# google/qhbm-library

Measured on AMD Instinct MI355X. Metric: circuit-expectation evals/sec (samples×Pauli terms) at n qubits; VQT step time, higher is better.
Workload: dtype f32; 1 GPU; BASELINE configs[2] (20-qubit XXZ, depth 16, 4096-sample VQT step): 20-qubit XXZ(delta=0.5) open chain, HEA depth 16 (944 params), 4096 states in total = 4096 on rank 0 of 1, VQT step = values + adjoint VJP; n_qubits=20, layers=16, states_total=4096, states_per_gpu=4096, pauli_terms=57, observables=1, hamiltonian=xxz, mode=vqt, parallelism=batch-sharded x1, backend_world_size=1, forward_passes=7, adjoint_passes=9

## Files before the change

qhbm-library_amd/csrc/engine.cpp:

```cpp
#include <hip/hip_runtime.h>

#include <algorithm>
#include <cmath>
#include <cstdio>
#include <iterator>
#include <cstdlib>
#include <cstring>
#include <memory>
#include <optional>
#include <string>
#include <vector>

#include "../../include/qhbm_engine.h"
#include "kernels.h"
#include "plan_args.h"
#include "program.h"
#include "schedule.h"

using namespace qhbm;

namespace {

std::string g_create_error;

// ... 55 lines not shown
};

struct TimedEvent {
  hipEvent_t a, b;
  int kind;
};

}

struct qhbm_engine {
  int device = -1;
  std::string err;
  Model model;
  bool have_circuit = false;
  int opt_tile = 0, opt_adj_tile = 0, opt_profile = 0, opt_round = 0;
  int opt_full_fwd = 60, opt_full_adj = 60, opt_force_general = 0;
  int opt_meas_tile = 0;
  int opt_values_from_obs = 1;
  bool retained_mu = false;
  int opt_cph_wave_bits = 1;
  int opt_fwd_values_obs = -1;
  int opt_adj_stop_early = -1;
  int opt_adj_plan_search = 1;
  int opt_wide_last = -1;
  int opt_fwd_pair = 1;
  int opt_shift_prefix = 1;
  int opt_adj_relabel = 1;
  int opt_obs_xcd_states = -1;
  int opt_x_two_shear = 1;
  int opt_adj_exchange = 1;
  int retained_U = 0;
  bool retained_table = false;
  int state_grad_U = 0;
  int64_t opt_chunk = 0;
  int64_t opt_budget_mb = 0;
  size_t resolved_budget = 0;
  bool plans_valid = false;
  bool adj_valid = false;
  std::vector<std::pair<std::vector<char>, std::unique_ptr<DevicePlan>>> adj_cache;
  int64_t fwd_plans_built = 0, adj_plans_built = 0;
  bool model_uploaded = false;
  DevicePlan fwd, adj;
  DevBuf<DevTerm> terms, global_terms;
  DevBuf<ObsGroup> obs_groups;
  bool terms_by_op = false;
  DevBuf<ObsBTerm> obs_bterms;
// ... 255 lines not shown

double pass_flops_per_amplitude(const Plan& plan, const Pass& p, const uint32_t* dyn = nullptr);

double adjoint_plan_seconds(const Plan& plan, const Model& m) {
  std::vector<PassArgs> args;
  std::vector<uint32_t> prog, tables;
  fill_args(plan, m, &args, &prog, &tables);
  const double amps = double(size_t(1) << plan.n_eff);
  double t = 0.0;
  for (size_t i = 0; i < args.size(); ++i) {
    const Pass& p = plan.passes[i];
    const double live = 1.0 / double(1ull << __builtin_popcount(args[i].zero_mask));
    int low_missing = 0;
    for (uint32_t k = 0; k < args[i].n_nonlocal; ++k) low_missing += args[i].nonlocal_pos[k] < 4;
    const double lines = std::min(1.0, live * double(1u << low_missing));
    const double write_share = (p.flags & PASS_RELABEL) ? 1.0 / double(1u << __builtin_popcount(p.frozen_new_local)) : 1.0;
    const double bytes = lines * amps * 8.0 * 2.0 * (1.0 + ((p.flags & PASS_STORE) ? write_share : 0.0));
    const double flops = live * amps * pass_flops_per_amplitude(plan, p);
    t += std::max(flops / 67e12, bytes / 5.5e12) + 0.1 * bytes / 5.5e12;
  }
  return t;
}

int build_plans(qhbm_engine* h) {
  if (h->plans_valid && h->adj_valid) return 0;
  if (!h->have_circuit) return fail(h, "qhbm_set_circuit has not been called");
  if (h->model.n_ops > kMaxOps) return fail(h, "too many observables (max 1024)");
  std::string err;
  if (!h->plans_valid) {
    h->adj_cache.clear();
    if (!build_plan(h->model, h->opt_tile, h->opt_round, false, &h->fwd.plan, &err, h->opt_full_fwd, h->opt_meas_tile,
                    h->opt_cph_wave_bits != 0, false, h->opt_wide_last))
      return fail(h, "forward plan: " + err);
    h->fwd.uploaded = false;
    ++h->fwd_plans_built;
  }
  const bool relabel = h->opt_adj_relabel != 0 && h->opt_adj_exchange != 0;
  auto plan_adjoint_of = [&](const Model& model, int tile, Plan* out, double* seconds, std::string* e) {
    if (!build_plan(model, tile, 0, true, out, e, h->opt_full_adj, 0, h->opt_cph_wave_bits != 0, relabel)) return false;
    *seconds = adjoint_plan_seconds(*out, model);
    if (!h->opt_adj_plan_search) return true;
    const std::vector<std::vector<uint32_t>> orders = out->candidate_orders;
    for (const std::vector<uint32_t>& order : orders) {
      Plan alt;
      std::string e2;
      if (!build_plan(model, tile, 0, true, &alt, &e2, h->opt_full_adj, 0, h->opt_cph_wave_bits != 0, relabel, -1, &order))
        continue;
      const double f = adjoint_plan_seconds(alt, model);
      if (std::getenv("QHBM_PLAN_DEBUG"))
        std::fprintf(stderr, "[plan] tile %d candidate with %zu passes: %.4g ms per state (kept so far: %zu passes, %.4g ms)\n", tile,
                     alt.passes.size(), f * 1e3, out->passes.size(), *seconds * 1e3);
      if (f < 0.99 * *seconds) { *out = std::move(alt); *seconds = f; }
    }
    return true;
  };
  auto plan_adjoint = [&](int tile, Plan* out, double* seconds, std::string* e) {
// ... 431 lines not shown
  HIPCHK(h->import_parts.reserve(import_norm_parts_count(n, c)));
  hipEvent_t* ev = timer_begin(h, 0, stream);
  HIPCHK(launch_import_states(h->import_src, n, n_eff, c, s0, h->psi.p, h->import_parts.p, h->import_norm2.p, stream));
  timer_end(ev, stream);
  if (h->import_upstream) {
    const size_t w = size_t(h->model.n_ops);
    HIPCHK(launch_scale_by_norm2(h->import_upstream + size_t(s0) * w, h->import_up.p + size_t(s0) * w, c, uint32_t(w),
                                 h->import_norm2.p + s0, stream));
  }
  return 0;
}

int run_forward_chunk(qhbm_engine* h, const int8_t* d_bits, uint32_t s0, uint32_t cs, bool keep_state,
                      hipStream_t stream, bool skip_measure = false) {
  DevicePlan& d = h->fwd;
  if (h->import_src)
    if (int rc = import_chunk(h, s0, cs, stream)) return rc;
  for (size_t i = 0; i < d.plan.passes.size(); ++i) {
    const Pass& p = d.plan.passes[i];
    if (skip_measure && p.is_measure_only) continue;
    const PassArgs a = forward_pass_args(h, i, keep_state, skip_measure);
    hipEvent_t* ev = timer_begin(h, 0, stream);
    const bool pair = h->opt_fwd_pair && cs >= 2 && !(a.flags & (PASS_INIT_BASIS | PASS_GENERAL)) && a.zero_mask == 0 &&
                      (skip_measure || p.n_meas_groups == 0) && pass_fwd_pair_supported(p.K);
    if (pair)
      HIPCHK(launch_pass_fwd_pair(p.K, a, cs, h->psi.p, d_bits, h->model.n, s0, d.prog.p, d.tables.p, d.coef.p, stream));
    else
      HIPCHK(launch_pass_fwd(p.K, d.plan.R, a, cs, h->psi.p, d_bits, h->model.n, d.prog.p, d.tables.p, d.coef.p,
                             h->op_scale.p, h->vals64.p, s0, stream));
    timer_end(ev, stream);
  }
  if (!d.plan.global_terms.empty() && !skip_measure)
    HIPCHK(launch_measure_global(h->psi.p, uint32_t(d.plan.n_eff), cs, h->global_terms.p,
                                 uint32_t(d.plan.global_terms.size()), h->op_scale.p, h->vals64.p,
                                 uint32_t(h->model.n_ops), s0, stream));
  return 0;
}

int values_begin(qhbm_engine* h, int U, hipStream_t stream) {
  const size_t nv = size_t(U) * size_t(std::max(h->model.n_ops, 1));
  HIPCHK(h->vals64.reserve(nv));
  HIPCHK(launch_zero_fill(h->vals64.p, nv * sizeof(unsigned long long), stream));
  return 0;
}
int values_end(qhbm_engine* h, int U, float* d_out, hipStream_t stream) {
  if (!d_out || h->model.n_ops <= 0) return 0;
// ... 500 lines not shown
  invalidate_plans(h);
  h->block_choice = -1;
  h->terms.release();
  return 0;
}

int qhbm_set_option(qhbm_engine* h, const char* name, int64_t value) {
  if (!h || !name) return 1;
  const std::string k(name);
  if (k == "tile_qubits") { h->opt_tile = int(value); invalidate_plans(h); h->block_choice = -1; }
  else if (k == "round_qubits") { h->opt_round = int(value); invalidate_plans(h); }
  else if (k == "force_general_kernels") h->opt_force_general = int(value);
  else if (k == "full_diag_threshold") { h->opt_full_fwd = int(value); invalidate_plans(h); }
  else if (k == "adjoint_full_diag_threshold") { h->opt_full_adj = int(value); invalidate_plans(h); }
  else if (k == "adjoint_tile_qubits") { h->opt_adj_tile = int(value); invalidate_plans(h); }
  else if (k == "adjoint_exchange") { h->opt_adj_exchange = int(value); invalidate_plans(h); }
  else if (k == "x_two_shear") { h->opt_x_two_shear = value != 0; invalidate_plans(h); h->adj_cache.clear(); h->dense.adj_cache.clear(); }
  else if (k == "adjoint_relabel") { h->opt_adj_relabel = int(value); invalidate_plans(h); }
  else if (k == "forward_pairs") h->opt_fwd_pair = int(value);
  else if (k == "shift_prefix_sharing") { h->opt_shift_prefix = int(value); h->shift_ready = false; }
  else if (k == "forward_values_from_observable") h->opt_fwd_values_obs = int(value);
  else if (k == "adjoint_stop_early") { h->opt_adj_stop_early = int(value); invalidate_plans(h); }
  else if (k == "adjoint_plan_search") { h->opt_adj_plan_search = int(value); invalidate_plans(h); }
  else if (k == "wide_last_pass") { h->opt_wide_last = int(value); invalidate_plans(h); }
  else if (k == "observable_xcd_states") h->opt_obs_xcd_states = int(value);
  else if (k == "observable_kernel") { h->opt_obs_kernel = int(value); h->block_choice = -1; }
  else if (k == "observable_split_rows") h->opt_obs_split_rows = value != 0;
  else if (k == "observable_block_bits") {
    if (value != kObsBlockBits && value != kObsBlockBitsSmall) return fail(h, "observable_block_bits: 12 or 13");
    h->opt_obs_block_bits = int(value); h->block_choice = -1; h->terms.release(); h->model_uploaded = false;
  }
  else if (k == "multi_observable_values") h->opt_multi_values = int(value);
  else if (k == "gather_multi_values") h->opt_gather_multi = int(value);
  else if (k == "observable_far_windows") { h->opt_far_windows = int(value); h->terms.release(); h->model_uploaded = false; }
  else if (k == "measure_tile_qubits") { h->opt_meas_tile = int(value); invalidate_plans(h); }
  else if (k == "values_from_observable") h->opt_values_from_obs = int(value);
  else if (k == "cph_wave_bits") { h->opt_cph_wave_bits = int(value); invalidate_plans(h); }
  else if (k == "chunk_states") h->opt_chunk = value;
  else if (k == "evolve_step_argument") {
    if (value < 1 || value > 64) return fail(h, "evolve_step_argument: 1 .. 64");
    h->opt_evolve_step = int(value);
  }
  else if (k == "workspace_budget_mb") h->opt_budget_mb = std::max<int64_t>(0, value);
  else if (k == "profile_events") h->opt_profile = int(value);
  else return fail(h, "unknown option '" + k + "'");
  return 0;
// ... 219 lines not shown
  if (int rc = prepare_coefs(h, d, d_params, -1, 0.0, s)) return rc;
  if (int rc = values_begin(h, U, s)) return rc;
  const uint32_t cs = chunk_states(h, U);
  if (int rc = ensure_state_buffers(h, cs, false)) return rc;
  const size_t row = size_t(8) << h->model.n, pitch = size_t(8) << d.plan.n_eff;
  for (uint32_t s0 = 0; s0 < uint32_t(U); s0 += cs) {
    const uint32_t c = std::min<uint32_t>(cs, uint32_t(U) - s0);
    if (int rc = h->model.gates.empty() ? import_chunk(h, s0, c, s) : run_forward_chunk(h, h->import_bits.p, s0, c, true, s)) return rc;
    char* out = static_cast<char*>(d_out_states) + size_t(s0) * row;
    HIPCHK(hipMemcpy2DAsync(out, row, h->psi.p, pitch, row, c, hipMemcpyDeviceToDevice, s));
    HIPCHK(launch_scale_state_rows(reinterpret_cast<float2*>(out), c, uint32_t(h->model.n), h->import_norm2.p + s0, s));
  }
  HIPCHK(h->phase_cs.reserve(2));
  HIPCHK(launch_global_phase(d.jobs.p, int(d.plan.jobs.size()), h->shift_phases.p, h->n_shift_phases, d_params,
                             h->phase_cs.p, s));
  HIPCHK(launch_scale_states(static_cast<float2*>(d_out_states), size_t(U) << h->model.n, h->phase_cs.p, s));
  return 0;
}

int qhbm_describe_schedule_from_states(qhbm_engine* h, char* buf, size_t buf_len) {
  if (!h || !buf || !buf_len) return 1;
  DenseScope scope(h);
  if (int rc = build_plans(h)) return rc;
  std::string s = describe_plan(h->fwd.plan) + describe_plan(h->adj.plan);
  char line[96];
  std::snprintf(line, sizeof(line), "adjoint time model: %.2f us per state\n", 1e6 * adjoint_plan_seconds(h->adj.plan, h->model));
  s += line;
  std::snprintf(buf, buf_len, "%s", s.c_str());
  return 0;
}

}

namespace {

struct EvolvePlan {
  double R = 0.0;
  int steps = 0;
  int terms = 0;
  double x = 0.0;
  std::vector<double> re, im;
};

std::vector<double> bessel_sequence(double x, int mode) {
  const int N = 2 * int(std::ceil(x)) + 64;
  std::vector<double> f(size_t(N) + 2, 0.0);
  f[size_t(N)] = 1.0;
// ... 746 lines not shown
  for (int k = 0; k < T; ++k) {
    for (size_t i = 0; i < nv; ++i) up[i] = (int(i % size_t(T)) == k) ? 1.f : 0.f;
    HIPCHK(hipMemcpyAsync(h->upstream_tmp.p, up.data(), nv * sizeof(float), hipMemcpyHostToDevice, s));
    HIPCHK(hipStreamSynchronize(s));
    if (int rc = adjoint_sweep(h, d_bits, U, d_params, h->upstream_tmp.p, d_out_vals, s)) return rc;
    HIPCHK(launch_scatter_jac(h->state_grad.p, uint32_t(U), uint32_t(h->adj.plan.slot_gate.size()),
                              h->param_slot_begin.p, h->param_slots.p, h->slot_factor.p, d_jac, uint32_t(T),
                              uint32_t(k), uint32_t(P), s));
  }
  return 0;
}

int qhbm_num_passes(qhbm_engine* h, int* forward_passes, int* backward_passes) {
  if (!h) return 1;
  if (int rc = build_plans(h)) return rc;
  if (forward_passes) *forward_passes = int(h->fwd.plan.passes.size());
  if (backward_passes) *backward_passes = int(h->adj.plan.passes.size());
  return 0;
}

int qhbm_describe_schedule(qhbm_engine* h, char* buf, size_t buf_len) {
  if (!h || !buf || !buf_len) return 1;
  if (int rc = build_plans(h)) return rc;
  std::string s = describe_plan(h->fwd.plan) + describe_plan(h->adj.plan);
  {
    char line[96];
    std::snprintf(line, sizeof(line), "adjoint time model: %.2f us per state\n", 1e6 * adjoint_plan_seconds(h->adj.plan, h->model));
    s += line;
  }
  if (!h->model.terms.empty()) {
    s += std::string("observable kernel: lambda = ") + (block_kernel(h) ? "observable_blocks_kernel" : "apply_observable_kernel");
    s += std::string(" values = ") + (gather_multi_mode(h) ? "apply_observable_kernel (an accumulator per observable)"
                                      : multi_value_mode(h) || (value_mode(h) && block_kernel(h)) ? "observable_blocks_kernel"
                                      : value_mode(h)                                            ? "apply_observable_kernel"
                                                                                                  : "measured in the passes");
    s += "\n";
  }
  std::snprintf(buf, buf_len, "%s", s.c_str());
  return 0;
}

int qhbm_kernel_time_ms(qhbm_engine* h, int reset, double* fwd_ms, int64_t* fwd_launches, double* bwd_ms,
                        int64_t* bwd_launches, double* obs_ms, int64_t* obs_launches) {
  if (!h) return 1;
  double ms[3] = {0.0, 0.0, 0.0};
  int64_t cnt[3] = {0, 0, 0};
  if (h->device >= 0 && !h->events.empty()) {
// ... 261 lines not shown
  if (obs_flops) *obs_flops = o;
  if (bwd_flops) *bwd_flops = b;
  return 0;
}

extern "C" {

int qhbm_traffic_model(qhbm_engine* h, int U, int with_vjp, double* fwd_bytes, double* obs_bytes,
                       double* bwd_bytes) {
  if (!h) return 1;
  if (int rc = build_plans(h)) return rc;
  const double tile_all = double(state_bytes(h)) * double(U);
  double f = 0.0, o = 0.0, b = 0.0;
  bool measure_only_after = !h->fwd.plan.global_terms.empty();
  for (const Pass& p : h->fwd.plan.passes) measure_only_after |= p.is_measure_only;
  const bool from_obs = with_vjp ? (value_mode(h) || multi_value_mode(h)) : forward_values_from_observable(h);
  {
    std::vector<PassArgs> fargs;
    std::vector<uint32_t> fprog, ftables;
    fill_args(h->fwd.plan, h->model, &fargs, &fprog, &ftables);
    for (size_t i = 0; i < fargs.size(); ++i) {
      const Pass& p = h->fwd.plan.passes[i];
      if (from_obs && p.is_measure_only) continue;
      const double live = 1.0 / double(1ull << __builtin_popcount(fargs[i].zero_mask));
      if (!(p.flags & PASS_INIT_BASIS)) f += live * tile_all;
      if (!p.is_measure_only && (!p.completes_circuit || from_obs || with_vjp || measure_only_after)) f += live * tile_all;
    }
  }
  if (!with_vjp && from_obs) o = tile_all;
  if (with_vjp) {
    o = 2.0 * tile_all;
    if (multi_value_mode(h) && !gather_multi_mode(h)) o += tile_all;
    std::vector<PassArgs> args;
    std::vector<uint32_t> prog, tables;
    fill_args(h->adj.plan, h->model, &args, &prog, &tables);
    for (size_t i = 0; i < args.size(); ++i) {
      double live = 1.0 / double(1ull << __builtin_popcount(args[i].zero_mask));
      {
        int low_missing = 0;
        for (uint32_t k = 0; k < args[i].n_nonlocal; ++k) low_missing += args[i].nonlocal_pos[k] < 4;
        live = std::min(1.0, live * double(1u << low_missing));
      }
      const Pass& ap = h->adj.plan.passes[i];
      double write_share = 1.0;
      if (ap.flags & PASS_RELABEL) write_share = 1.0 / double(1u << __builtin_popcount(ap.frozen_new_local));
      b += live * tile_all * 2.0 * (1.0 + ((ap.flags & PASS_STORE) ? write_share : 0.0));
    }
// ... 9 lines not shown
```

qhbm-library_amd/csrc/kernels.hip:

```cpp
#include <hip/hip_runtime.h>
#include <stdint.h>
#include <cstdio>
#include <cstring>

#include <utility>

#include "../../include/qhbm_engine.h"
#include "device_common.h"
#include "kernels.h"
#include "program.h"
#include "x_shear.h"

namespace qhbm {

namespace {


__device__ __forceinline__ uint32_t swz(uint32_t l) { return l ^ ((l >> 5) & 31u); }

constexpr int wg_per_cu(int lds_bytes) { return (160 * 1024) / lds_bytes < 1 ? 1 : (160 * 1024) / lds_bytes; }
constexpr int clampi(int v, int lo, int hi) { return v < lo ? lo : (v > hi ? hi : v); }
constexpr int fwd_lds(int K) { return (8 << K) + 8 * kMaxOps; }
constexpr int adj_lds(int K) { return (16 << K) + 4 * kMaxSlotsPerPass * ((1 << (K - 4)) / 64 < 1 ? 1 : (1 << (K - 4)) / 64); }
constexpr int adjx_lds(int K) { return (8 << K) + 4 * kMaxSlotsPerPass * ((1 << (K - 4)) / 64 < 1 ? 1 : (1 << (K - 4)) / 64); }
// ... 887 lines not shown
  wht_lane_stage<3>(w, lane);
  wht_lane_stage<4>(w, lane);
  wht_lane_stage<5>(w, lane);
  uint32_t begin = 0;
#pragma unroll
  for (int c = 0; c < NR; ++c) {
    const uint32_t end = uni(class_end[c]);
    if (end != begin) {
      scr[lane] = w[c];
      for (uint32_t k = begin + uint32_t(lane); k < end; k += 64u) {
        const uint32_t* tw = terms + size_t(k) * kMeasTermWords;
        const uint4 t = make_uint4(tw[0], tw[1], tw[2], tw[3]);
        const uint32_t par = uint32_t(__popc(tile_base & t.y) + __popc(wave & (t.x >> 6))) & 1u;
        const float v = __uint_as_float(t.z ^ (par << 31)) * scr[t.x & 63u];
        atomicAdd(&red[t.w], to_fixed(v, op_scale[t.w]));
      }
    }
    begin = end;
  }
}

}

template <int K, int R, bool GEN>
__global__ __launch_bounds__(1 << (K - R), fwd_min_waves(K, R)) void pass_fwd_kernel(
    PassArgs a, float2* __restrict__ psi, const int8_t* __restrict__ bits, int n_user,
    const uint32_t* __restrict__ prog_base, const uint32_t* __restrict__ tables,
    const float* __restrict__ coef, const float* __restrict__ op_scale, unsigned long long* __restrict__ out64,
    uint32_t state0, const float2* __restrict__ psi_src) {
  constexpr int NT = 1 << (K - R);
  constexpr int NR = 1 << R;
  extern __shared__ __attribute__((aligned(16))) unsigned char smem[];
  float2* tile = reinterpret_cast<float2*>(smem);
  unsigned long long* red = reinterpret_cast<unsigned long long*>(tile + (1 << K));

  const int tid = threadIdx.x;
  const int lane = tid & 63;
  const uint32_t s_local = blockIdx.x >> a.n_free;
  uint32_t bits_row = state0 + s_local, out_row = state0 + s_local;
  if (a.prog_states) {
    const uint32_t q = s_local / a.prog_states;
    bits_row = state0 + (s_local - q * a.prog_states);
    out_row = s_local;
    coef += size_t(q) * a.coef_stride;
  }
  const uint32_t* recs = reinterpret_cast<const uint32_t*>(coef);
  TileCtx t = pass_tile_ctx(a, tables);
  const ThreadOff toff = thread_offsets(t, tid);
  uint32_t idx = 0;
  if ((a.flags & PASS_INIT_BASIS) | a.zero_mask | a.frozen_old_local) idx = input_index(a, bits + size_t(bits_row) * n_user, n_user, lane);
  const uint32_t in_local = local_bits<K>(a, idx, lane);
  const uint32_t tile_id = launched_tile(a, blockIdx.x, idx, lane);
  t.tile_base = tile_base_of(a, tile_id, lane);
  const uint32_t tile_hi = tile_id << K;
  float2* st = psi + (size_t(s_local) << a.n);

  if (a.flags & PASS_INIT_BASIS) {
    if ((idx & a.nonlocal_mask) != t.tile_base) {
      if ((a.flags & PASS_STORE) && !(a.flags & PASS_NO_ZERO_FILL)) {
        for (int p = tid; p < (1 << (K - 1)); p += NT)
          *reinterpret_cast<float4*>(st + global_index(t, 2u * p)) = make_float4(0.f, 0.f, 0.f, 0.f);
      }
      return;
    }
    for (int l = tid; l < (1 << K); l += NT) tile[l] = make_float2(0.f, 0.f);
    __syncthreads();
    if (tid == 0) tile[swz(in_local)] = make_float2(1.f, 0.f);
  } else {
    TileRegs r;
    const float2* ld = psi_src ? psi_src + (size_t(bits_row - state0) << a.n) : st;
    prefetch_tile<K, NT>(r, ld, t, toff);
    if (a.frozen_old_local) clear_stale<K>(r, tid, in_local, a.frozen_old_local);
    commit_tile<K, NT>(tile, r, tid);
  }
  for (int i = tid; i < kMaxOps; i += NT) red[i] = 0ull;
  __syncthreads();

  const uint32_t* prog = prog_base + a.prog_off;
  uint32_t pc = 0;
  constexpr int NV = 1;
  uint32_t cur[NV], nxt[NV];
  uint32_t carried_off = 0xffffffffu;
  for (;;) {
    const uint32_t w0 = uni(prog[pc]);
    const uint32_t opc = w0 & 0xffu;
    if (opc == OP_END) break;
    if (opc == OP_ROUND) {
      const uint32_t n_inst = (w0 & ~kRoundNoBarrier) >> 8;
      const uint32_t regmask = uni(prog[pc + 1]);
      uint32_t rec_off = uni(prog[pc + 2]);
      constexpr RecordLayout L(R, false);
      if (rec_off != carried_off) rec_load<NV>(recs, rec_off, lane, cur);
      uint32_t DB[R], T;
      const uint32_t TL = tables[a.tl_off + uni(prog[pc + 3]) + uint32_t(tid)];
// ... 75 lines not shown
          const uint32_t key = zhi | ((ny & 1u) << 16);
          if (key != last_key) {
            sum = (ny & 1) ? meas_sum<R, 1>(w, zhi) : meas_sum<R, 0>(w, zhi);
            last_key = key;
          }
          acc = fmaf(sfac, sum, acc);
        }
      }
      if (cur_op != 0xffffffffu) {
        const float v = wave_sum(acc);
        if ((tid & 63) == 0) atomicAdd(&red[cur_op], to_fixed(v, op_scale[cur_op]));
      }
      __syncthreads();
    }
  }

  if (a.n_ops) {
    __syncthreads();
    for (uint32_t i = tid; i < a.n_ops; i += NT) {
      const unsigned long long v = red[i];
      if (v) atomicAdd(&out64[size_t(out_row) * a.n_ops + i], v);
    }
  }
  if (a.flags & PASS_STORE) store_tile<K, NT>(tile, st, t, thread_offsets(t, tid), tid);
}

template <int K>
__global__ __launch_bounds__(1 << (K - 4), adjx_min_waves(K)) void pass_fwd2_kernel(
    PassArgs a, float2* __restrict__ psi, const int8_t* __restrict__ bits, int n_user, uint32_t state0,
    const uint32_t* __restrict__ prog_base, const uint32_t* __restrict__ tables, const float* __restrict__ coef,
    uint32_t n_states) {
  constexpr int R = 4;
  constexpr int NT = 1 << (K - R);
  constexpr int NR = 1 << R;
  extern __shared__ __attribute__((aligned(16))) unsigned char smem[];
  float2* xt = reinterpret_cast<float2*>(smem);
  lds_tile_at_zero(smem);
  const int tid = threadIdx.x;
  const int lane = tid & 63;
  const uint32_t* recs = reinterpret_cast<const uint32_t*>(coef);
  const uint32_t tile_id = blockIdx.x & ((1u << a.n_nonlocal) - 1u);
  const uint32_t pair = blockIdx.x >> a.n_nonlocal;
  const uint32_t s_a = 2u * pair, s_b = min(2u * pair + 1u, n_states - 1u);
  TileCtx t = pass_tile_ctx(a, tables);
  const ThreadOff toff = thread_offsets(t, tid);
  t.tile_base = tile_base_of(a, tile_id, lane);
  const uint32_t tile_hi = tile_id << K;
// ... 1083 lines not shown
}

constexpr int kMaxDevices = 64;
size_t fwd_lds_bytes(int K) { return size_t(fwd_lds(K)); }
size_t adj_lds_bytes(int K, bool exchange) { return size_t(exchange ? adjx_lds(K) : adj_lds(K)); }

template <typename Kernel>
static hipError_t opt_in_lds(Kernel kernel, bool (&done)[kMaxDevices], size_t lds) {
  int dev = 0;
  if (hipError_t e = hipGetDevice(&dev); e != hipSuccess) return e;
  if (dev < 0 || dev >= kMaxDevices || !done[dev]) {
    hipError_t e = hipFuncSetAttribute(reinterpret_cast<const void*>(kernel),
                                       hipFuncAttributeMaxDynamicSharedMemorySize, int(lds));
    if (e != hipSuccess) return e;
    if (dev >= 0 && dev < kMaxDevices) done[dev] = true;
  }
  return hipSuccess;
}

static bool pass_prologue_ok(int K, const PassArgs& a, int n_user) {
  return K >= 10 && n_user >= 1 && n_user <= 32 && a.n >= 1u && a.n <= 32u && a.n_nonlocal <= 32u;
}

template <int K, int R, bool GEN>
static hipError_t launch_fwd_t(const PassArgs& a, uint32_t n_states, float2* psi, const int8_t* bits,
                               int n_user, const uint32_t* prog, const uint32_t* tables,
                               const float* coef, const float* op_scale, unsigned long long* out64, uint32_t state0,
                               hipStream_t stream, const float2* psi_src) {
  const size_t lds = fwd_lds_bytes(K);
  static bool attr_done[kMaxDevices] = {};
  if (hipError_t e = opt_in_lds(&pass_fwd_kernel<K, R, GEN>, attr_done, lds); e != hipSuccess) return e;
  const uint32_t grid = n_states << a.n_free;
  hipLaunchKernelGGL((pass_fwd_kernel<K, R, GEN>), dim3(grid), dim3(1 << (K - R)), lds, stream, a, psi, bits,
                     n_user, prog, tables, coef, op_scale, out64, state0, psi_src);
  return hipGetLastError();
}

hipError_t launch_pass_fwd(int K, int R, const PassArgs& a, uint32_t n_states, float2* psi, const int8_t* bits,
                           int n_user, const uint32_t* prog, const uint32_t* tables, const float* coef,
                           const float* op_scale, unsigned long long* out64, uint32_t state0, hipStream_t stream,
                           const float2* psi_src) {
  if (!pass_prologue_ok(K, a, n_user)) return hipErrorInvalidValue;
  if (psi_src && ((a.flags & PASS_INIT_BASIS) || !a.prog_states)) return hipErrorInvalidValue;
#define QHBM_FWD_CASE(K_, R_)                                                                          \
  if (K == K_ && R == R_)                                                                              \
    return (a.flags & PASS_GENERAL)                                                                    \
               ? launch_fwd_t<K_, R_, true>(a, n_states, psi, bits, n_user, prog, tables, coef, op_scale, out64, state0, stream, psi_src)   \
               : launch_fwd_t<K_, R_, false>(a, n_states, psi, bits, n_user, prog, tables, coef, op_scale, out64, state0, stream, psi_src);
  QHBM_FWD_CASE(10, 4)
  QHBM_FWD_CASE(11, 4)
  QHBM_FWD_CASE(12, 4)
  QHBM_FWD_CASE(13, 4)
  QHBM_FWD_CASE(14, 4)
#undef QHBM_FWD_CASE
  return hipErrorInvalidValue;
}
// ... 857 lines not shown
```

qhbm-library_amd/csrc/schedule.cpp:

```cpp
#include "schedule.h"

#include <algorithm>
#include <cmath>
#include <cstdio>
#include <cstdlib>
#include <cstring>
#include <sstream>

#include "../../include/qhbm_engine.h"

namespace qhbm {
namespace {

inline int popc(uint32_t x) { return __builtin_popcount(x); }

bool odd_constant(const Gate& G) {
  if (G.param_idx >= 0) return false;
  const float t = G.offset;
  return t == std::nearbyint(t) && (long(std::nearbyint(t)) & 1L);
}

bool lower(const Model& m, std::vector<LoweredOp>* ops, std::string* err, double* const_phase = nullptr,
           std::vector<std::pair<int, float>>* phases = nullptr) {
  ops->clear();
// ... 703 lines not shown
        uint32_t cb;
        std::memcpy(&cb, &t.coeff, 4);
        p->prog.push_back(to_local(*p, t.z & S));
        p->prog.push_back(t.z & ~S);
        p->prog.push_back(cb);
        p->prog.push_back(uint32_t(t.op) | (uint32_t(t.ny & 3) << 24));
        ++p->n_meas_terms;
      }
      ++p->n_meas_groups;
    }
  }

 private:
  const Model& m_;
  int K_, R_, n_eff_;
  bool adjoint_;
  Plan* plan_;
};

}

bool build_plan(const Model& m, int tile_bits, int round_bits, bool adjoint, Plan* plan, std::string* err,
                int full_threshold, int meas_tile_bits, bool cph_wave_bits, bool relabel, int wide_last_pass,
                const std::vector<uint32_t>* forced_order) {
  *plan = Plan();
  plan->full_threshold = full_threshold;
  plan->cph_wave_bits = cph_wave_bits;
  plan->tail_tiles = cph_wave_bits;
  if (m.n < 1 || m.n > kMaxQubits - 1) { *err = "n_qubits must be in [1, 31]"; return false; }
  const int n_eff = std::max(m.n, kMinTileBits);
  const int k_cap = adjoint ? kMaxTileBits - 1 : kMaxTileBits;
  int K;
  if (tile_bits == 0) {
    K = n_eff <= k_cap ? n_eff : (adjoint || n_eff <= 21 ? 12 : 13);
  } else {
    if (tile_bits < kMinTileBits || tile_bits > k_cap) {
      *err = "tile_qubits out of range";
      return false;
    }
    K = std::min(n_eff, tile_bits);
  }
  const int R = kRoundBits;
  if (round_bits != 0 && round_bits != kRoundBits) {
    *err = "round_qubits must be 4";
    return false;
  }
  plan->n = m.n;
// ... 272 lines not shown
      size_t best_total = 0;
      uint32_t best_set = 0;
      std::vector<int> best;
      for (uint32_t S : gen_cands(dn, gphys)) {
        int n_mat = 0;
        std::vector<int> lst = absorb_capped(dn, S, &n_mat);
        if (n_mat > best_mat || (n_mat == best_mat && lst.size() > best_total)) { best_mat = n_mat; best_total = lst.size(); best_set = S; best.swap(lst); }
      }
      if (best.empty()) break;
      for (int oi : best) dn[size_t(oi)] = 1;
      left -= best.size();
      ++greedy_passes;
      greedy_sets.push_back(best_set);
      if (plan->relabel && left) relabel_after(best_set, dn, &gphys, &gfrozen);
    }
    std::sort(complete.begin(), complete.end(), [](const auto& x, const auto& y) { return x.first < y.first; });
    for (const auto& c : complete) {
      if (plan->candidate_orders.size() >= 6) break;
      if (c.second != planned) plan->candidate_orders.push_back(c.second);
    }
    if (left == 0) plan->candidate_orders.push_back(greedy_sets);
    if (left == 0 && planned.size() > greedy_passes + (plan->relabel ? 4 : 1)) planned.clear();
  }
  size_t planned_i = 0;
  {
    if (const char* env = std::getenv(adjoint ? "QHBM_ADJ_SETS" : "QHBM_FWD_SETS")) {
      planned.clear();
      for (const char* q = env; *q;) {
        char* end = nullptr;
        const unsigned long v = std::strtoul(q, &end, 16);
        if (end == q) break;
        planned.push_back(uint32_t(v));
        q = *end ? end + 1 : end;
      }
    }
  }

  while (n_done < ops.size()) {
    std::vector<uint32_t> cands = planned_i < planned.size() ? std::vector<uint32_t>{planned[planned_i++]} : gen_cands(done, phys);
    int wide_K = 0;
    uint32_t wide_S = 0;
    const bool widen = wide_last_pass > 0 || (wide_last_pass < 0 && tile_bits == 0);
    if (!adjoint && K < n_eff && plan->tail_tiles && widen && !plan->passes.empty() && !std::getenv("QHBM_NO_WIDE_LAST_PASS")) {
      uint32_t S = (1u << c_min) - 1;
      for (int oi : order) {
        if (done[oi]) continue;
        const LoweredOp& op = ops[oi];
        S |= op.type == LOW_DIAG ? (op.bits & S ? 0u : (op.bits & (0u - op.bits))) : op.bits;
      }
      const int need = popc(S);
      if (need > K && need <= std::min(K + 2, std::min(n_eff, 13))) {
        wide_K = need;
        wide_S = S;
      }
    }
    if (!adjoint && K < n_eff && !groups.empty()) {
      uint32_t S = (1u << c_min) - 1;
      bool fits = true;
      for (int oi : order) {
        if (done[oi]) continue;
        const LoweredOp& op = ops[oi];
        const uint32_t need = op.type == LOW_DIAG ? (op.bits & S ? 0u : (op.bits & (0u - op.bits))) : op.bits;
        if (popc(S | need) > K) { fits = false; break; }
        S |= need;
      }
      if (fits) {
        const int here = int(plan->passes.size());
        for (size_t gi = 0; gi < groups.size() && fits; ++gi) {
          const int ready = group_ready(gi, here);
          bool earlier = false;
          for (int pi = ready; pi < here && !earlier; ++pi) earlier = (groups[gi].x & ~pass_set(plan->passes[size_t(pi)])) == 0;
          if (earlier) continue;
          if (popc(S | groups[gi].x) <= K) S |= groups[gi].x; else fits = false;
        }
      }
      if (fits) {
        for (int bit = n_eff - 1; bit >= 0 && popc(S) < K; --bit) if (!(S >> bit & 1)) S |= 1u << bit;
        cands.insert(cands.begin(), S);
      }
    }
    uint32_t best_S = 0;
    int best_mat = -1;
    size_t best_total = 0;
    std::vector<int> best_list;
    std::vector<uint32_t> blocks;
    if (K < n_eff) {
      const uint32_t low = (1u << c_min) - 1;
      const int h = K - c_min;
      for (int pp = c_min; pp + h <= n_eff; ++pp) blocks.push_back(low | (((1u << h) - 1) << pp));
    }
    for (uint32_t S : cands) {
      int n_mat = 0;
      std::vector<int> lst = absorb_capped(done, S, &n_mat);
      int next_best = 0;
      if (!adjoint && !blocks.empty() && n_done + lst.size() < ops.size()) {
        std::vector<char> done2(done);
        for (int oi : lst) done2[oi] = 1;
        for (uint32_t S2 : blocks) {
          int m2 = 0;
          absorb(ops, order, done2, S2, all_bits, &m2);
          next_best = std::max(next_best, m2);
        }
      }
      const int score = n_mat + next_best;
      if (score > best_mat || (score == best_mat && lst.size() > best_total)) {
        best_mat = score; best_total = lst.size(); best_S = S; best_list.swap(lst);
      }
    }
    if (best_list.empty()) { *err = "scheduler made no progress"; return false; }
    Builder wide(m, wide_K ? wide_K : K, R, n_eff, adjoint, plan);
    Builder* bp = &b;
    if (wide_K) {
      int n_mat = 0;
      std::vector<int> all_left = absorb(ops, order, done, wide_S, all_bits, &n_mat);
// ... 350 lines not shown
```

qhbm-library_amd/csrc/schedule.h:

```cpp
#pragma once
#include <cstdint>
#include <string>
#include <vector>

#include "program.h"

namespace qhbm {

struct Gate {
  int32_t kind, q0, q1, param_idx;
  float scalar, offset;
  float global_shift;
};

struct PauliTerm {
  float coeff;
  uint32_t x, z;
  int ny;
  int op;
};

struct LoweredOp {
  int type = LOW_SKIP;
  int kind = 0;
// ... 41 lines not shown
  std::vector<uint32_t> round_wavemasks;
  std::vector<uint32_t> round_words;
  int n_meas_groups = 0, n_meas_terms = 0;
  int slot_base = 0, n_slots = 0;
  uint32_t mat_bits = 0;
};

struct Plan {
  int n = 0, n_eff = 0, K = 0, R = 0;
  bool adjoint = false;
  std::vector<Pass> passes;
  std::vector<CoefJob> jobs;
  int n_coef_floats = 0;
  std::vector<uint32_t> coef_init;
  std::vector<uint32_t> record_offsets;
  int full_threshold = 60;
  bool tail_tiles = true;
  bool relabel = false;
  bool cph_wave_bits = true;
  std::vector<int> global_terms;
  std::vector<int> slot_gate;
  std::vector<float> slot_factor;
  std::vector<std::vector<uint32_t>> candidate_orders;
  bool dense_tail = false;
  bool dense_input = false;
  double const_phase = 0.0;
  std::vector<std::pair<int, float>> gate_phases;
};

struct Model {
  int n = 0;
  int n_params = 0;
  std::vector<Gate> gates;
  std::vector<char> param_frozen;
  bool stop_at_first_live_gate = true;
  bool frozen(int param_idx) const { return param_idx >= 0 && size_t(param_idx) < param_frozen.size() && param_frozen[size_t(param_idx)]; }
  int n_ops = 0;
  std::vector<PauliTerm> terms;
  bool dense_input = false;
};


bool build_plan(const Model& m, int tile_bits, int round_bits, bool adjoint, Plan* out,
                std::string* err, int full_threshold = 60, int meas_tile_bits = 0, bool cph_wave_bits = true,
                bool relabel = false, int wide_last_pass = -1, const std::vector<uint32_t>* forced_order = nullptr);

std::string describe_plan(const Plan& p);

std::vector<int> first_dependent_pass(const Plan& plan, size_t n_gates, int* first_measuring);

struct ProgramOrder {
  std::vector<int> dst;
  std::vector<uint32_t> group_end;
  bool shares = false;
};
ProgramOrder order_programs(const Plan& fwd, size_t n_gates, const int* shift_gates, size_t n_programs, bool may_share,
                            bool values_outside_passes);

}
```

Measured before the change: 732,400 evals/s.

## Add beam-search forward plan selection and ROWS8 kernel for c==0 passes

Adds an optional forward-plan search: a beam search over tile bit sets plus reversed adjoint orders, scored by an analytic time model, with forced-order plan building in the scheduler. Forward passes with c==0 now launch a ROWS8 kernel variant and no longer use the paired-state kernel. The forward cost estimate also accounts for low nonlocal bits when computing live lines. The plan search is off by default, so the default path changes only through the kernel routing and the estimator.

Result: no change. 730,900 evals/s (-0.2%).

```diff
diff --git a/qhbm-library_amd/csrc/engine.cpp b/qhbm-library_amd/csrc/engine.cpp
--- a/qhbm-library_amd/csrc/engine.cpp
+++ b/qhbm-library_amd/csrc/engine.cpp
@@ -101,6 +101,7 @@
   int opt_fwd_values_obs = -1;
   int opt_adj_stop_early = -1;
   int opt_adj_plan_search = 1;
+  int opt_fwd_plan_search = 0;
   int opt_wide_last = -1;
   int opt_fwd_pair = 1;
   int opt_shift_prefix = 1;
@@ -402,6 +403,116 @@
   return t;
 }
 
+constexpr double kFwdRate = 108e12;
+constexpr double kFwdFixed = 1.05e-6;
+constexpr double kFwdSingle = 1.13;
+constexpr double kFwdSingle8 = 1.84;
+double forward_plan_seconds(const Plan& plan, const Model& m, std::string* detail = nullptr) {
+  std::vector<PassArgs> args;
+  std::vector<uint32_t> prog, tables;
+  fill_args(plan, m, &args, &prog, &tables);
+  const double amps = double(size_t(1) << plan.n_eff);
+  double t = 0.0;
+  for (size_t i = 0; i < args.size(); ++i) {
+    const Pass& p = plan.passes[i];
+    const double live = 1.0 / double(1ull << __builtin_popcount(args[i].zero_mask));
+    const bool first = (p.flags & PASS_INIT_BASIS) != 0;
+    const double share = first ? 1.0 / double(1ull << p.nonlocal_pos.size()) : live;
+    const bool pair = !first && !(p.flags & PASS_GENERAL) && args[i].zero_mask == 0 && args[i].c != 0 && !p.is_measure_only && pass_fwd_pair_supported(p.K);
+    int low_missing = 0;
+    for (uint32_t k = 0; k < args[i].n_nonlocal; ++k) low_missing += args[i].nonlocal_pos[k] < 4;
+    const double lines = std::min(1.0, live * double(1u << low_missing));
+    const double bytes = amps * 8.0 * ((first ? 0.0 : lines) + (p.is_measure_only ? 0.0 : lines));
+    const double flops = share * amps * pass_flops_per_amplitude(plan, p);
+    const double pass_t = std::max(share * kFwdFixed + flops / kFwdRate * (pair ? 1.0 : (args[i].c == 0 ? kFwdSingle8 : kFwdSingle)), bytes / 5.5e12);
+    if (detail) {
+      char b[96];
+      std::snprintf(b, sizeof(b), "%s%.3g%s", i ? " " : "", 1e6 * pass_t, pair ? "" : (p.is_measure_only ? "m" : "s"));
+      *detail += b;
+    }
+    t += pass_t;
+  }
+  return t;
+}
+
+bool plan_forward(qhbm_engine* h, Plan* out, std::string* err) {
+  std::string text;
+  std::string* report = &text;
+  auto build = [&](Plan* pl, std::string* e, const std::vector<uint32_t>* order, bool search) {
+    return build_plan(h->model, h->opt_tile, h->opt_round, false, pl, e, h->opt_full_fwd, h->opt_meas_tile,
+                      h->opt_cph_wave_bits != 0, false, h->opt_wide_last, order, search);
+  };
+  if (!build(out, err, nullptr, h->opt_fwd_plan_search != 0)) return false;
+  if (!h->opt_fwd_plan_search) return true;
+  char line[256];
+  if (out->K >= out->n_eff || h->model.dense_input || !h->opt_cph_wave_bits) {
+    *report = std::string("forward plan search: greedy plan kept (") +
+              (out->K >= out->n_eff ? "one tile holds the state" : h->model.dense_input ? "a caller-supplied start state prunes nothing" : "cph_wave_bits=0") + ")\n";
+    out->search_report = text;
+    return true;
+  }
+  struct Cand { std::string name; std::vector<uint32_t> order; };
+  std::vector<Cand> cands;
+  for (size_t i = 0; i < out->candidate_orders.size(); ++i) cands.push_back(Cand{"search #" + std::to_string(i), out->candidate_orders[i]});
+  {
+    Model whole = h->model;
+    whole.param_frozen.clear();
+    Plan adj;
+    std::string e2;
+    const bool relabel = h->opt_adj_relabel != 0 && h->opt_adj_exchange != 0;
+    if (out->K <= kMaxTileBits - 1 && build_plan(whole, out->K, 0, true, &adj, &e2, h->opt_full_adj, 0, h->opt_cph_wave_bits != 0, relabel)) {
+      std::vector<std::vector<uint32_t>> orders;
+      std::vector<uint32_t> own;
+      for (const Pass& p : adj.passes) { uint32_t S = 0; for (int b : p.local_pos) S |= 1u << b; own.push_back(S); }
+      orders.push_back(own);
+      for (const auto& o : adj.candidate_orders) orders.push_back(o);
+      for (size_t i = 0; i < orders.size(); ++i)
+        cands.push_back(Cand{"backward order #" + std::to_string(i) + ", reversed", std::vector<uint32_t>(orders[i].rbegin(), orders[i].rend())});
+    }
+  }
+  std::string detail;
+  double best = forward_plan_seconds(*out, h->model, &detail);
+  const double greedy = best;
+  std::snprintf(line, sizeof(line), "forward plan search: greedy %zu passes, %.2f us per state [%s]\n", out->passes.size(), 1e6 * greedy, detail.c_str());
+  *report += line;
+  std::string kept = "greedy";
+  const bool need_no_zero_fill = !out->passes.empty() && (out->passes[0].flags & PASS_NO_ZERO_FILL);
+  const size_t greedy_global = out->global_terms.size(), n_greedy_passes = out->passes.size();
+  std::vector<std::vector<uint32_t>> seen;
+  for (const Cand& c : cands) {
+    if (std::find(seen.begin(), seen.end(), c.order) != seen.end()) {
+      *report += "  " + c.name + ": same order as an earlier candidate\n";
+      continue;
+    }
+    seen.push_back(c.order);
+    Plan alt;
+    std::string e2;
+    if (!build(&alt, &e2, &c.order, false)) {
+      *report += "  " + c.name + ": not admissible (" + e2 + ")\n";
+      continue;
+    }
+    if ((need_no_zero_fill && !(alt.passes[0].flags & PASS_NO_ZERO_FILL)) || alt.global_terms.size() > greedy_global) {
+      *report += "  " + c.name + ": greedy kept (the order breaks a precondition of prefix sharing or of the tile measurement)\n";
+      continue;
+    }
+    if (alt.passes.size() > n_greedy_passes && h->opt_fwd_plan_search != 2) {
+      std::snprintf(line, sizeof(line), ": %zu passes, more than the greedy plan: greedy kept\n", alt.passes.size());
+      *report += "  " + c.name + line;
+      continue;
+    }
+    detail.clear();
+    const double f = forward_plan_seconds(alt, h->model, &detail);
+    std::snprintf(line, sizeof(line), ": %zu passes, %.2f us per state [%s]\n", alt.passes.size(), 1e6 * f, detail.c_str());
+    *report += "  " + c.name + line;
+    const bool first_forced = h->opt_fwd_plan_search == 2 && kept == "greedy";
+    if (f < 0.99 * best || first_forced) { *out = std::move(alt); best = f; kept = c.name; }
+  }
+  std::snprintf(line, sizeof(line), "  kept: %s (%.2f us per state, greedy %.2f)\n", kept.c_str(), 1e6 * best, 1e6 * greedy);
+  *report += line;
+  out->search_report = text;
+  return true;
+}
+
 int build_plans(qhbm_engine* h) {
   if (h->plans_valid && h->adj_valid) return 0;
   if (!h->have_circuit) return fail(h, "qhbm_set_circuit has not been called");
@@ -409,9 +520,7 @@
   std::string err;
   if (!h->plans_valid) {
     h->adj_cache.clear();
-    if (!build_plan(h->model, h->opt_tile, h->opt_round, false, &h->fwd.plan, &err, h->opt_full_fwd, h->opt_meas_tile,
-                    h->opt_cph_wave_bits != 0, false, h->opt_wide_last))
-      return fail(h, "forward plan: " + err);
+    if (!plan_forward(h, &h->fwd.plan, &err)) return fail(h, "forward plan: " + err);
     h->fwd.uploaded = false;
     ++h->fwd_plans_built;
   }
@@ -889,6 +998,7 @@
     const PassArgs a = forward_pass_args(h, i, keep_state, skip_measure);
     hipEvent_t* ev = timer_begin(h, 0, stream);
     const bool pair = h->opt_fwd_pair && cs >= 2 && !(a.flags & (PASS_INIT_BASIS | PASS_GENERAL)) && a.zero_mask == 0 &&
+                      a.c != 0 &&
                       (skip_measure || p.n_meas_groups == 0) && pass_fwd_pair_supported(p.K);
     if (pair)
       HIPCHK(launch_pass_fwd_pair(p.K, a, cs, h->psi.p, d_bits, h->model.n, s0, d.prog.p, d.tables.p, d.coef.p, stream));
@@ -1435,6 +1545,7 @@
   else if (k == "forward_values_from_observable") h->opt_fwd_values_obs = int(value);
   else if (k == "adjoint_stop_early") { h->opt_adj_stop_early = int(value); invalidate_plans(h); }
   else if (k == "adjoint_plan_search") { h->opt_adj_plan_search = int(value); invalidate_plans(h); }
+  else if (k == "forward_plan_search") { h->opt_fwd_plan_search = int(value); invalidate_plans(h); }
   else if (k == "wide_last_pass") { h->opt_wide_last = int(value); invalidate_plans(h); }
   else if (k == "observable_xcd_states") h->opt_obs_xcd_states = int(value);
   else if (k == "observable_kernel") { h->opt_obs_kernel = int(value); h->block_choice = -1; }
@@ -1700,7 +1811,7 @@
   if (!h || !buf || !buf_len) return 1;
   DenseScope scope(h);
   if (int rc = build_plans(h)) return rc;
-  std::string s = describe_plan(h->fwd.plan) + describe_plan(h->adj.plan);
+  std::string s = describe_plan(h->fwd.plan) + h->fwd.plan.search_report + describe_plan(h->adj.plan);
   char line[96];
   std::snprintf(line, sizeof(line), "adjoint time model: %.2f us per state\n", 1e6 * adjoint_plan_seconds(h->adj.plan, h->model));
   s += line;
@@ -2493,7 +2604,7 @@
 int qhbm_describe_schedule(qhbm_engine* h, char* buf, size_t buf_len) {
   if (!h || !buf || !buf_len) return 1;
   if (int rc = build_plans(h)) return rc;
-  std::string s = describe_plan(h->fwd.plan) + describe_plan(h->adj.plan);
+  std::string s = describe_plan(h->fwd.plan) + h->fwd.plan.search_report + describe_plan(h->adj.plan);
   {
     char line[96];
     std::snprintf(line, sizeof(line), "adjoint time model: %.2f us per state\n", 1e6 * adjoint_plan_seconds(h->adj.plan, h->model));
@@ -2801,7 +2912,12 @@
     for (size_t i = 0; i < fargs.size(); ++i) {
       const Pass& p = h->fwd.plan.passes[i];
       if (from_obs && p.is_measure_only) continue;
-      const double live = 1.0 / double(1ull << __builtin_popcount(fargs[i].zero_mask));
+      double live = 1.0 / double(1ull << __builtin_popcount(fargs[i].zero_mask));
+      {
+        int low_missing = 0;
+        for (uint32_t k = 0; k < fargs[i].n_nonlocal; ++k) low_missing += fargs[i].nonlocal_pos[k] < 4;
+        live = std::min(1.0, live * double(1u << low_missing));
+      }
       if (!(p.flags & PASS_INIT_BASIS)) f += live * tile_all;
       if (!p.is_measure_only && (!p.completes_circuit || from_obs || with_vjp || measure_only_after)) f += live * tile_all;
     }
diff --git a/qhbm-library_amd/csrc/kernels.hip b/qhbm-library_amd/csrc/kernels.hip
--- a/qhbm-library_amd/csrc/kernels.hip
+++ b/qhbm-library_amd/csrc/kernels.hip
@@ -933,7 +933,7 @@
 
 }
 
-template <int K, int R, bool GEN>
+template <int K, int R, bool GEN, int ROWS = ROWS16>
 __global__ __launch_bounds__(1 << (K - R), fwd_min_waves(K, R)) void pass_fwd_kernel(
     PassArgs a, float2* __restrict__ psi, const int8_t* __restrict__ bits, int n_user,
     const uint32_t* __restrict__ prog_base, const uint32_t* __restrict__ tables,
@@ -957,7 +957,7 @@
   }
   const uint32_t* recs = reinterpret_cast<const uint32_t*>(coef);
   TileCtx t = pass_tile_ctx(a, tables);
-  const ThreadOff toff = thread_offsets(t, tid);
+  const ThreadOff toff = thread_offsets<ROWS>(t, tid);
   uint32_t idx = 0;
   if ((a.flags & PASS_INIT_BASIS) | a.zero_mask | a.frozen_old_local) idx = input_index(a, bits + size_t(bits_row) * n_user, n_user, lane);
   const uint32_t in_local = local_bits<K>(a, idx, lane);
@@ -969,8 +969,12 @@
   if (a.flags & PASS_INIT_BASIS) {
     if ((idx & a.nonlocal_mask) != t.tile_base) {
       if ((a.flags & PASS_STORE) && !(a.flags & PASS_NO_ZERO_FILL)) {
-        for (int p = tid; p < (1 << (K - 1)); p += NT)
-          *reinterpret_cast<float4*>(st + global_index(t, 2u * p)) = make_float4(0.f, 0.f, 0.f, 0.f);
+        if constexpr (ROWS == ROWS8) {
+          for (int l = tid; l < (1 << K); l += NT) st[global_index(t, uint32_t(l))] = make_float2(0.f, 0.f);
+        } else {
+          for (int p = tid; p < (1 << (K - 1)); p += NT)
+            *reinterpret_cast<float4*>(st + global_index(t, 2u * p)) = make_float4(0.f, 0.f, 0.f, 0.f);
+        }
       }
       return;
     }
@@ -980,7 +984,7 @@
   } else {
     TileRegs r;
     const float2* ld = psi_src ? psi_src + (size_t(bits_row - state0) << a.n) : st;
-    prefetch_tile<K, NT>(r, ld, t, toff);
+    prefetch_tile<K, NT, ROWS>(r, ld, t, toff);
     if (a.frozen_old_local) clear_stale<K>(r, tid, in_local, a.frozen_old_local);
     commit_tile<K, NT>(tile, r, tid);
   }
@@ -1102,7 +1106,7 @@
       if (v) atomicAdd(&out64[size_t(out_row) * a.n_ops + i], v);
     }
   }
-  if (a.flags & PASS_STORE) store_tile<K, NT>(tile, st, t, thread_offsets(t, tid), tid);
+  if (a.flags & PASS_STORE) store_tile<K, NT, ROWS>(tile, st, t, thread_offsets<ROWS>(t, tid), tid);
 }
 
 template <int K>
@@ -2232,16 +2236,19 @@
   return K >= 10 && n_user >= 1 && n_user <= 32 && a.n >= 1u && a.n <= 32u && a.n_nonlocal <= 32u;
 }
 
-template <int K, int R, bool GEN>
+template <int K, int R, bool GEN, int ROWS = ROWS16>
 static hipError_t launch_fwd_t(const PassArgs& a, uint32_t n_states, float2* psi, const int8_t* bits,
                                int n_user, const uint32_t* prog, const uint32_t* tables,
                                const float* coef, const float* op_scale, unsigned long long* out64, uint32_t state0,
                                hipStream_t stream, const float2* psi_src) {
   const size_t lds = fwd_lds_bytes(K);
   static bool attr_done[kMaxDevices] = {};
-  if (hipError_t e = opt_in_lds(&pass_fwd_kernel<K, R, GEN>, attr_done, lds); e != hipSuccess) return e;
+  if constexpr (ROWS == ROWS16) {
+    if (a.c == 0) return launch_fwd_t<K, R, GEN, ROWS8>(a, n_states, psi, bits, n_user, prog, tables, coef, op_scale, out64, state0, stream, psi_src);
+  }
+  if (hipError_t e = opt_in_lds(&pass_fwd_kernel<K, R, GEN, ROWS>, attr_done, lds); e != hipSuccess) return e;
   const uint32_t grid = n_states << a.n_free;
-  hipLaunchKernelGGL((pass_fwd_kernel<K, R, GEN>), dim3(grid), dim3(1 << (K - R)), lds, stream, a, psi, bits,
+  hipLaunchKernelGGL((pass_fwd_kernel<K, R, GEN, ROWS>), dim3(grid), dim3(1 << (K - R)), lds, stream, a, psi, bits,
                      n_user, prog, tables, coef, op_scale, out64, state0, psi_src);
   return hipGetLastError();
 }
diff --git a/qhbm-library_amd/csrc/schedule.cpp b/qhbm-library_amd/csrc/schedule.cpp
--- a/qhbm-library_amd/csrc/schedule.cpp
+++ b/qhbm-library_amd/csrc/schedule.cpp
@@ -749,7 +749,7 @@
 
 bool build_plan(const Model& m, int tile_bits, int round_bits, bool adjoint, Plan* plan, std::string* err,
                 int full_threshold, int meas_tile_bits, bool cph_wave_bits, bool relabel, int wide_last_pass,
-                const std::vector<uint32_t>* forced_order) {
+                const std::vector<uint32_t>* forced_order, bool forward_search) {
   *plan = Plan();
   plan->full_threshold = full_threshold;
   plan->cph_wave_bits = cph_wave_bits;
@@ -1068,9 +1068,137 @@
     if (left == 0) plan->candidate_orders.push_back(greedy_sets);
     if (left == 0 && planned.size() > greedy_passes + (plan->relabel ? 4 : 1)) planned.clear();
   }
+
+  const uint32_t low_bits = (1u << c_min) - 1u;
+  if (!adjoint && forward_search && !forced_order && K < n_eff && plan->tail_tiles && !m.dense_input && !ops.empty() &&
+      !std::getenv("QHBM_FWD_SETS")) {
+    struct Node { std::vector<char> dn; size_t n_done; double cost; std::vector<uint32_t> sets; };
+    double kFixed = 11.5, kMemory = 36.0, kSingle = 1.31;
+    if (const char* e = std::getenv("QHBM_FWD_PLAN_KFIXED")) kFixed = std::atof(e);
+    if (const char* e = std::getenv("QHBM_FWD_PLAN_KMEMORY")) kMemory = std::atof(e);
+    size_t kBeam = ops.size() <= 4000 ? 16 : (ops.size() <= 12000 ? 8 : 4);
+    if (const char* e = std::getenv("QHBM_FWD_PLAN_BEAM")) kBeam = size_t(std::max(1, std::atoi(e)));
+    const std::vector<int> rorder(order.rbegin(), order.rend());
+    auto mirror_cands = [&](const std::vector<char>& dn) {
+      std::vector<uint32_t> cs;
+      const int h = K - c_min;
+      for (int p = c_min; p + h <= n_eff; ++p) cs.push_back(low_bits | (((1u << h) - 1) << p));
+      const uint32_t pending_mat = pending_mat_of(dn);
+      const uint32_t low_live = low_bits & pending_mat;
+      if (low_live != low_bits) {
+        const int h2 = K - popc(low_live);
+        std::vector<int> ub;
+        for (int bit = c_min; bit < n_eff; ++bit) if (pending_mat >> bit & 1u) ub.push_back(bit);
+        for (size_t p0 = 0; p0 + size_t(h2) <= ub.size(); ++p0) {
+          uint32_t S = low_live;
+          for (int k = 0; k < h2; ++k) S |= 1u << ub[p0 + size_t(k)];
+          cs.push_back(S);
+        }
+      }
+      for (int with_diag = 0; with_diag < 2; ++with_diag) {
+        uint32_t S = low_live, blocked = 0;
+        for (int oi : rorder) {
+          if (dn[size_t(oi)]) continue;
+          const LoweredOp& op = ops[size_t(oi)];
+          if (op.bits & blocked) { blocked |= op.bits; continue; }
+          if (op.type == LOW_DIAG && !with_diag) continue;
+          if (popc(S | op.bits) <= K) S |= op.bits; else blocked |= op.bits;
+        }
+        for (int bit = n_eff - 1; bit >= 0 && popc(S) < K; --bit) if (!(S >> bit & 1)) S |= 1u << bit;
+        cs.push_back(S);
+      }
+      std::sort(cs.begin(), cs.end());
+      cs.erase(std::unique(cs.begin(), cs.end()), cs.end());
+      return cs;
+    };
+    std::vector<std::pair<double, std::vector<uint32_t>>> found;
+    std::vector<Node> beam(1);
+    beam[0].dn.assign(ops.size(), 0);
+    beam[0].n_done = 0;
+    beam[0].cost = 0.0;
+    double best_cost = -1.0;
+    for (int depth = 0; depth < 256 && !beam.empty(); ++depth) {
+      std::vector<Node> next;
+      for (const Node& nd : beam) {
+        for (uint32_t S : mirror_cands(nd.dn)) {
+          int n_mat = 0;
+          std::vector<int> lst = absorb(ops, rorder, nd.dn, S, all_bits, &n_mat);
+          if (lst.empty()) continue;
+          Node c;
+          c.dn = nd.dn;
+          for (int oi : lst) c.dn[size_t(oi)] = 1;
+          c.n_done = nd.n_done + lst.size();
+          const uint32_t untouched = all_bits & ~pending_mat_of(c.dn);
+          const double alive = 1.0 / double(1u << std::min(20, popc(untouched & ~S)));
+          const double work = kFixed + double(n_mat) * (alive < 1.0 ? kSingle : 1.0);
+          const double lines = std::min(1.0, alive * double(1u << popc(low_bits & ~S)));
+          c.cost = nd.cost + std::max(kMemory * lines, alive * work);
+          c.sets = nd.sets;
+          c.sets.push_back(S);
+          if (c.n_done == ops.size()) {
+            found.emplace_back(c.cost, c.sets);
+            if (best_cost < 0.0 || c.cost < best_cost) best_cost = c.cost;
+            continue;
+          }
+          bool dup = false;
+          for (Node& o : next)
+            if (o.n_done == c.n_done && o.dn == c.dn) { dup = true; if (c.cost < o.cost) o = c; break; }
+          if (!dup) next.push_back(std::move(c));
+        }
+      }
+      auto rank = [&](const Node& nd) {
+        size_t mats_left = 0;
+        for (size_t oi = 0; oi < ops.size(); ++oi) mats_left += !nd.dn[oi] && ops[oi].type != LOW_DIAG;
+        const int nfin = std::min(4, popc(all_bits & ~pending_mat_of(nd.dn) & ~low_bits));
+        return nd.cost + double(mats_left) / double(1 << nfin);
+      };
+      std::vector<std::pair<double, size_t>> keyed;
+      for (size_t i = 0; i < next.size(); ++i) keyed.emplace_back(rank(next[i]), i);
+      std::sort(keyed.begin(), keyed.end());
+      std::vector<Node> kept;
+      for (size_t i = 0; i < keyed.size() && kept.size() < kBeam; ++i) {
+        Node& nd = next[keyed[i].second];
+        if (best_cost >= 0.0 && nd.cost >= best_cost) continue;
+        kept.push_back(std::move(nd));
+      }
+      beam.swap(kept);
+    }
+    std::sort(found.begin(), found.end(), [](const auto& x, const auto& y) { return x.first < y.first; });
+    for (const auto& f : found) {
+      if (plan->candidate_orders.size() >= 4) break;
+      std::vector<uint32_t> fwd_sets(f.second.rbegin(), f.second.rend());
+      if (std::find(plan->candidate_orders.begin(), plan->candidate_orders.end(), fwd_sets) == plan->candidate_orders.end())
+        plan->candidate_orders.push_back(std::move(fwd_sets));
+    }
+  }
+  std::vector<std::vector<int>> lazy_lists;
+  if (!adjoint && forced_order) {
+    if (K >= n_eff || planned.empty()) { *err = "forced order: the plan has one pass"; return false; }
+    const std::vector<int> rorder(order.rbegin(), order.rend());
+    std::vector<char> dn(ops.size(), 0);
+    lazy_lists.resize(planned.size());
+    size_t got = 0;
+    for (size_t i = planned.size(); i-- > 0;) {
+      const uint32_t S = planned[i];
+      if ((S & ~all_bits) || popc(S) != K) {
+        *err = "forced order: a tile holds exactly tile_bits index bits";
+        return false;
+      }
+      int n_mat = 0;
+      std::vector<int> lst = absorb(ops, rorder, dn, S, all_bits, &n_mat);
+      for (int oi : lst) dn[size_t(oi)] = 1;
+      got += lst.size();
+      std::sort(lst.begin(), lst.end());
+      lazy_lists[i].swap(lst);
+    }
+    if (got != ops.size()) { *err = "forced order: it does not cover the circuit"; return false; }
+    plan->forced = true;
+  }
+  size_t lazy_i = 0;
   size_t planned_i = 0;
   {
-    if (const char* env = std::getenv(adjoint ? "QHBM_ADJ_SETS" : "QHBM_FWD_SETS")) {
+    const char* env = forced_order && !adjoint ? nullptr : std::getenv(adjoint ? "QHBM_ADJ_SETS" : "QHBM_FWD_SETS");
+    if (env) {
       planned.clear();
       for (const char* q = env; *q;) {
         char* end = nullptr;
@@ -1083,7 +1211,13 @@
   }
 
   while (n_done < ops.size()) {
-    std::vector<uint32_t> cands = planned_i < planned.size() ? std::vector<uint32_t>{planned[planned_i++]} : gen_cands(done, phys);
+    const bool lazy = !lazy_lists.empty();
+    if (lazy) {
+      while (lazy_i < lazy_lists.size() && lazy_lists[lazy_i].empty()) ++lazy_i;
+      if (lazy_i >= lazy_lists.size()) { *err = "internal: forced order ran out of passes"; return false; }
+    }
+    std::vector<uint32_t> cands = lazy ? std::vector<uint32_t>{planned[lazy_i]}
+                                  : planned_i < planned.size() ? std::vector<uint32_t>{planned[planned_i++]} : gen_cands(done, phys);
     int wide_K = 0;
     uint32_t wide_S = 0;
     const bool widen = wide_last_pass > 0 || (wide_last_pass < 0 && tile_bits == 0);
@@ -1100,7 +1234,7 @@
         wide_S = S;
       }
     }
-    if (!adjoint && K < n_eff && !groups.empty()) {
+    if (!adjoint && K < n_eff && !groups.empty() && !lazy) {
       uint32_t S = (1u << c_min) - 1;
       bool fits = true;
       for (int oi : order) {
@@ -1135,7 +1269,13 @@
       const int h = K - c_min;
       for (int pp = c_min; pp + h <= n_eff; ++pp) blocks.push_back(low | (((1u << h) - 1) << pp));
     }
+    if (lazy) {
+      best_S = planned[lazy_i];
+      best_list = lazy_lists[lazy_i];
+      ++lazy_i;
+    }
     for (uint32_t S : cands) {
+      if (lazy) break;
       int n_mat = 0;
       std::vector<int> lst = absorb_capped(done, S, &n_mat);
       int next_best = 0;
diff --git a/qhbm-library_amd/csrc/schedule.h b/qhbm-library_amd/csrc/schedule.h
--- a/qhbm-library_amd/csrc/schedule.h
+++ b/qhbm-library_amd/csrc/schedule.h
@@ -87,6 +87,8 @@
   std::vector<int> slot_gate;
   std::vector<float> slot_factor;
   std::vector<std::vector<uint32_t>> candidate_orders;
+  bool forced = false;
+  std::string search_report;
   bool dense_tail = false;
   bool dense_input = false;
   double const_phase = 0.0;
@@ -108,7 +110,8 @@
 
 bool build_plan(const Model& m, int tile_bits, int round_bits, bool adjoint, Plan* out,
                 std::string* err, int full_threshold = 60, int meas_tile_bits = 0, bool cph_wave_bits = true,
-                bool relabel = false, int wide_last_pass = -1, const std::vector<uint32_t>* forced_order = nullptr);
+                bool relabel = false, int wide_last_pass = -1, const std::vector<uint32_t>* forced_order = nullptr,
+                bool forward_search = false);
 
 std::string describe_plan(const Plan& p);
 
```
